# arindamrc/video_analytics

Hardware: AMD Instinct MI355X
Metric: clips/sec (224x224, RGB+10-flow two-stream) (higher is better)
Workload: dtype f32; 1 GPU; two-stream 224x224, 10-frame TV-L1 flow stack (5 scales x 5 warps x 300 its, fixed), VGG-16 spatial+temporal, batch=32 per GPU; global_batch=32, block_iters=0, tvl1_math=exact, flow_streams=2, batches_in_flight=1, tvl1_params=, tvl1_hip_blob=2e95b55cc558928abf4903d3eda147c92736cfdd, parallelism=clips sharded x1, finite=True

## Files before the change

video_analytics_amd/csrc/vgg.hip:

```cpp
#include "vgg_internal.h"
#include <cstdint>
#include <cstdlib>
#include <cstring>
#include <type_traits>

namespace {

typedef float f32x16 __attribute__((ext_vector_type(16)));
typedef float f32x4 __attribute__((ext_vector_type(4)));
typedef unsigned u32x4 __attribute__((ext_vector_type(4)));

template <int N, typename F>
__device__ __forceinline__ void static_for(F&& f)
{
    if constexpr (N > 0) {
        static_for<N - 1>(f);
        f(std::integral_constant<int, N - 1>{});
    }
}

constexpr int kBK = 16;
constexpr int kLdsStride = 20;


// ... 938 lines not shown
            constexpr int i = decltype(I)::value;
            if ((wave * PPW + i) < NPIECE) {
                const int y = Y0 + (pyx[i] >> 8) - 1, x = X0 + (pyx[i] & 255) - 1;
                const bool ok = pyx[i] >= 0 && y >= 0 && y < H && x >= 0 && x < W;
                __builtin_amdgcn_raw_ptr_buffer_load_lds(rs_a, (lds_ptr_t)(sA + buf * A_BYTES + (wave * PPW + i) * 1024), 16,
                                                         ok ? base + rel[i] : 0x7fffffff, 0, 0, 0);
            }
        });
    };

    const int r31 = lane & 31, hh = lane >> 5;
    int idx0[2], px0[2], py0[2];
#pragma unroll
    for (int mt = 0; mt < 2; ++mt) {
        int xl, yl, bl;
        brick_coords(64 * wave + 32 * mt + r31, 4, 4, xl, yl, bl);
        px0[mt] = xl + 1;
        py0[mt] = yl + 1;
        idx0[mt] = py0[mt] * PW + px0[mt];
    }
    const char* const wfrag = sW + r31 * WSTRIDE + hh * 16;

    if (first < aw.n_bricks) stage_a(first, 0);
    asm volatile("s_waitcnt vmcnt(0) lgkmcnt(0)" ::: "memory");
    __syncthreads();

    int buf = 0;
    for (int brick = first; brick < aw.n_bricks; brick += stride) {
        if (brick + stride < aw.n_bricks) stage_a(brick + stride, buf ^ 1);
        f32x16 acc[2][2];
#pragma unroll
        for (int mt = 0; mt < 2; ++mt)
#pragma unroll
            for (int nt = 0; nt < 2; ++nt)
#pragma unroll
                for (int r = 0; r < 16; ++r) acc[mt][nt][r] = 0.0f;
        const char* const pA = sA + buf * A_BYTES;
        bf16x8 fa[3][2], fb[3][2];
        auto fetch = [&](int i, int slot) __attribute__((always_inline)) {
            const int tap = i >> 2, ks = i & 3;
            const int toff = (tap / 3 - 1) * PW + (tap % 3) - 1;
#pragma unroll
            for (int mt = 0; mt < 2; ++mt) {
                const int row = idx0[mt] + toff;
                const int sw = (((px0[mt] + (tap % 3) - 1) >> 1) + 4 * (py0[mt] + tap / 3 - 1)) & 7;
                fa[slot][mt] = *reinterpret_cast<const bf16x8*>(pA + row * 128 + (((2 * ks + hh) ^ sw) << 4));
            }
#pragma unroll
            for (int nt = 0; nt < 2; ++nt)
                fb[slot][nt] = *reinterpret_cast<const bf16x8*>(wfrag + nt * 32 * WSTRIDE + (tap * 64 + ks * 16) * 2);
        };
        fetch(0, 0);
        fetch(1, 1);
#pragma unroll
        for (int i = 0; i < 36; ++i) {
            if (i + 2 < 36) fetch(i + 2, (i + 2) % 3);
            __builtin_amdgcn_sched_barrier(0);
#pragma unroll
            for (int mt = 0; mt < 2; ++mt)
#pragma unroll
                for (int nt = 0; nt < 2; ++nt)
                    acc[mt][nt] = kWeightsFirst<POOL> ? __builtin_amdgcn_mfma_f32_32x32x16_bf16(fb[i % 3][nt], fa[i % 3][mt], acc[mt][nt], 0, 0, 0)
                                                      : __builtin_amdgcn_mfma_f32_32x32x16_bf16(fa[i % 3][mt], fb[i % 3][nt], acc[mt][nt], 0, 0, 0);
            __builtin_amdgcn_sched_barrier(0);
        }
        asm volatile("s_waitcnt lgkmcnt(0)" ::: "memory");
        __builtin_amdgcn_s_barrier();
        {
            const int tx = brick % a.tiles_x, r1 = brick / a.tiles_x, ty = r1 % a.tiles_y, b = r1 / a.tiles_y;
            epilogue_lines_bf16<2, POOL>(acc, (__bf16*)(sA + buf * A_BYTES) + wave * 64 * 64, a, 64 * wave, nb, tx << 4, ty << 4, b, lane);
        }
        asm volatile("s_waitcnt vmcnt(0) lgkmcnt(0)" ::: "memory");
        __builtin_amdgcn_s_barrier();
        buf ^= 1;
    }
}

template <bool POOL>
__global__ void __launch_bounds__(256) k_conv3x3_ws_bf16(ConvArgsWs a)
{
    conv3x3_ws_body<POOL>(a);
}

struct Img14Args {
    const void* in;
    const void* wp;
    const float* bias;
    void* out;
    int B, Cin, Cout;
};

template <typename T, bool POOL>
__device__ __forceinline__ void conv3x3_img14_body(const Img14Args& a)
{
    constexpr bool F32 = sizeof(T) == 4;
    constexpr int EPC = 16 / (int)sizeof(T);
    constexpr int BK = 8 * EPC;
    constexpr int BRICK = 256 * BK, WT = 3 * 64 * BK, NWR = 3;
    constexpr int WPIECES = 6, BPIECES = 8;
    __shared__ __attribute__((aligned(1024))) T smem[2 * BRICK + NWR * WT];
    T* const sBrick = smem;
    T* const sW = smem + 2 * BRICK;
    const int tid = threadIdx.x, lane = tid & 63;
    const int wave8 = __builtin_amdgcn_readfirstlane(tid >> 6);
    const int wave = wave8 & 3;
    const int tiles_n = a.Cout / 64;
    const int n_tile = blockIdx.x % tiles_n, b = blockIdx.x / tiles_n;
    const int n0 = n_tile * 64, Cin = a.Cin;
    const int r31 = lane & 31, hh = lane >> 5, lrow = lane >> 3, lslot = lane & 7;
    const int nchunks = Cin / BK, NT_STEPS = 3 * nchunks;
    auto brick_swz = [](int bp) { return ((bp >> 1) & 3) | (((bp >> 4) & 1) << 2); };

    if (wave8 >= 4) {
        const T* const in = (const T*)a.in;
        const T* const wp = (const T*)a.wp;
        const __amdgpu_buffer_rsrc_t rs_a = __builtin_amdgcn_make_buffer_rsrc(
            const_cast<T*>(in) + (size_t)b * 196 * Cin, 0, 196 * Cin * (int)sizeof(T), 0x00020000);
        const __amdgpu_buffer_rsrc_t rs_b = __builtin_amdgcn_make_buffer_rsrc(
            const_cast<T*>(wp) + (size_t)n0 * 9 * Cin, 0, 64 * 9 * Cin * (int)sizeof(T), 0x00020000);
        int aoff[BPIECES];
#pragma unroll
        for (int i = 0; i < BPIECES; ++i) {
            const int bp = ((wave * 8 + i) << 3) + lrow, by = bp >> 4, bx = bp & 15;
            const bool ok = by >= 1 && by <= 14 && bx >= 1 && bx <= 14;
            aoff[i] = ok ? (((by - 1) * 14 + (bx - 1)) * Cin + EPC * (lslot ^ brick_swz(bp))) * (int)sizeof(T) : 0x7fffffff;
        }
        int boff[2];
#pragma unroll
        for (int i = 0; i < 2; ++i) {
            const int row = (wave * 2 + i) * 8 + lrow;
            boff[i] = (row * 9 * Cin + EPC * (lslot ^ ((row >> 1) & 7))) * (int)sizeof(T);
        }
        auto stage_brick = [&](int chunk) {
            T* const dst = sBrick + (chunk & 1) * BRICK;
            static_for<BPIECES>([&](auto I) {
                constexpr int i = decltype(I)::value;
                __builtin_amdgcn_raw_ptr_buffer_load_lds(rs_a, (lds_ptr_t)(dst + (wave * 8 + i) * 8 * BK), 16, aoff[i], chunk * BK * (int)sizeof(T), 0, 0);
            });
        };
        auto stage_w = [&](int t) {
            const int chunk = t / 3, ky = t - 3 * chunk;
            T* const dst = sW + (t % NWR) * WT;
            static_for<WPIECES>([&](auto I) {
                constexpr int i = decltype(I)::value, kx = i >> 1, h = i & 1;
                __builtin_amdgcn_raw_ptr_buffer_load_lds(rs_b, (lds_ptr_t)(dst + kx * 64 * BK + (wave * 2 + h) * 8 * BK), 16, boff[h],
                                                         ((3 * ky + kx) * Cin + chunk * BK) * (int)sizeof(T), 0, 0);
            });
        };
        stage_brick(0);
        stage_w(0);
        if (NT_STEPS > 1) stage_w(1);
        bool brick_prev = false;
        for (int t = 0; t < NT_STEPS; ++t) {
            const int chunk = t / 3, ky = t - 3 * chunk;
            if (t + 1 >= NT_STEPS) asm volatile("s_waitcnt vmcnt(0)" ::: "memory");
            else if (brick_prev) asm volatile("s_waitcnt vmcnt(14)" ::: "memory");
            else asm volatile("s_waitcnt vmcnt(6)" ::: "memory");
            __builtin_amdgcn_s_barrier();
            brick_prev = ky == 0 && chunk + 1 < nchunks;
            if (brick_prev) stage_brick(chunk + 1);
            if (t + 2 < NT_STEPS) stage_w(t + 2);
        }
        return;
    }

    constexpr int MT = 2, NT = 2;
    typedef typename std::conditional<F32, f32x4, bf16x8>::type frag_t;
    const int nrb = wave < 3 ? 2 : 1;
    int bp0[MT];
#pragma unroll
    for (int i = 0; i < MT; ++i) {
        const int qy = wave + 4 * i, qx = r31 >> 2;
        const int y = 2 * qy + ((r31 >> 1) & 1), x = 2 * qx + (r31 & 1);
        bp0[i] = (qx < 7 && qy < 7) ? (y + 1) * 16 + (x + 1) : 0;
    }
    f32x16 acc[MT][NT];
#pragma unroll
    for (int i = 0; i < MT; ++i)
#pragma unroll
        for (int j = 0; j < NT; ++j)
#pragma unroll
            for (int r = 0; r < 16; ++r) acc[i][j][r] = 0.0f;
    const int fsw = (r31 >> 1) & 7;
    auto mma = [&](const frag_t& fpix, const frag_t& fwgt, f32x16& c) __attribute__((always_inline)) {
        if constexpr (F32) {
#pragma unroll
            for (int e = 0; e < 4; ++e)
                c = POOL ? __builtin_amdgcn_mfma_f32_32x32x2f32(fpix[e], fwgt[e], c, 0, 0, 0) : __builtin_amdgcn_mfma_f32_32x32x2f32(fwgt[e], fpix[e], c, 0, 0, 0);
        } else {
            c = POOL ? __builtin_amdgcn_mfma_f32_32x32x16_bf16(fpix, fwgt, c, 0, 0, 0) : __builtin_amdgcn_mfma_f32_32x32x16_bf16(fwgt, fpix, c, 0, 0, 0);
        }
    };

    for (int t = 0; t < NT_STEPS; ++t) {
        const int chunk = t / 3, ky = t - 3 * chunk;
        asm volatile("s_waitcnt lgkmcnt(0)" ::: "memory");
        __builtin_amdgcn_s_barrier();
        const T* const sA = sBrick + (chunk & 1) * BRICK;
        const T* const sB = sW + (t % NWR) * WT;
        int arow[3][MT], asw[3][MT];
#pragma unroll
        for (int kx = 0; kx < 3; ++kx)
#pragma unroll
            for (int i = 0; i < MT; ++i) {
                const int bp = bp0[i] ? bp0[i] + (ky - 1) * 16 + (kx - 1) : 0;
                arow[kx][i] = bp * BK;
                asw[kx][i] = brick_swz(bp);
            }
        frag_t fa[2][2][MT], fb[2][2][NT];
        auto fetch = [&](auto SS, auto BUF) {
            constexpr int ss = decltype(SS)::value, kx = ss >> 1, bf = decltype(BUF)::value;
#pragma unroll
            for (int h = 0; h < 2; ++h) {
                const int ks = 2 * (ss & 1) + h;
#pragma unroll
                for (int i = 0; i < MT; ++i) fa[bf][h][i] = *reinterpret_cast<const frag_t*>(&sA[arow[kx][i] + (((2 * ks + hh) ^ asw[kx][i]) * EPC)]);
#pragma unroll
                for (int j = 0; j < NT; ++j)
                    fb[bf][h][j] = *reinterpret_cast<const frag_t*>(&sB[kx * 64 * BK + (j * 32 + r31) * BK + (((2 * ks + hh) ^ fsw) * EPC)]);
            }
        };
        fetch(std::integral_constant<int, 0>{}, std::integral_constant<int, 0>{});
        static_for<6>([&](auto SS) {
            constexpr int ss = decltype(SS)::value, cur = ss & 1;
            if constexpr (ss + 1 < 6) fetch(std::integral_constant<int, ss + 1>{}, std::integral_constant<int, cur ^ 1>{});
            __builtin_amdgcn_sched_barrier(0);
#pragma unroll
            for (int h = 0; h < 2; ++h)
#pragma unroll
                for (int i = 0; i < MT; ++i)
#pragma unroll
                    for (int j = 0; j < NT; ++j) mma(fa[cur][h][i], fb[cur][h][j], acc[i][j]);
            __builtin_amdgcn_sched_barrier(0);
        });
    }

    if constexpr (POOL) {
        float* const out = (float*)a.out + (size_t)b * 49 * a.Cout;
#pragma unroll
        for (int i = 0; i < MT; ++i) {
            if (i >= nrb) continue;
#pragma unroll
            for (int j = 0; j < NT; ++j) {
                const int n = n0 + 32 * j + r31;
                const float bias = a.bias[n];
#pragma unroll
                for (int g4 = 0; g4 < 4; ++g4) {
                    const int qy = wave + 4 * i, qx = 2 * g4 + hh;
                    if (qx >= 7 || qy >= 7) continue;
                    const int quad = 7 * qy + qx;
                    const float m01 = fmaxf(acc[i][j][4 * g4 + 0], acc[i][j][4 * g4 + 1]), m23 = fmaxf(acc[i][j][4 * g4 + 2], acc[i][j][4 * g4 + 3]);
                    out[(size_t)quad * a.Cout + n] = fmaxf(fmaxf(m01, m23) + bias, 0.0f);
                }
            }
        }
    } else {
        constexpr int NCHK = 64 / EPC;
        T* const stage = sBrick + (nchunks & 1) * BRICK + wave * 32 * 64;
        T* const out = (T*)a.out + (size_t)b * 196 * a.Cout + n0;
#pragma unroll
        for (int i = 0; i < MT; ++i) {
            if (i >= nrb) continue;
            const int qy = wave + 4 * i;
#pragma unroll
            for (int j = 0; j < NT; ++j)
#pragma unroll
                for (int g4 = 0; g4 < 4; ++g4) {
                    const int n = 32 * j + 8 * g4 + 4 * hh;
                    const float4 bs = *(const float4*)(a.bias + n0 + n);
                    const float v0 = fmaxf(acc[i][j][4 * g4 + 0] + bs.x, 0.0f), v1 = fmaxf(acc[i][j][4 * g4 + 1] + bs.y, 0.0f);
                    const float v2 = fmaxf(acc[i][j][4 * g4 + 2] + bs.z, 0.0f), v3 = fmaxf(acc[i][j][4 * g4 + 3] + bs.w, 0.0f);
                    T* const dst = stage + r31 * 64 + (((n / EPC) ^ (r31 & (NCHK - 1))) * EPC) + (n % EPC);
                    if constexpr (F32) {
                        *(float4*)dst = make_float4(v0, v1, v2, v3);
                    } else {
                        typedef __bf16 bf16x4 __attribute__((ext_vector_type(4)));
                        bf16x4 v;
                        v.x = (__bf16)v0, v.y = (__bf16)v1, v.z = (__bf16)v2, v.w = (__bf16)v3;
                        *(bf16x4*)dst = v;
                    }
                }
            __builtin_amdgcn_wave_barrier();
#pragma unroll
            for (int it = 0; it < 32 * NCHK / 64; ++it) {
                const int ch = it * 64 + lane, r = ch / NCHK, c8 = ch % NCHK, qx = r >> 2;
                const uint4 v = *(const uint4*)(stage + r * 64 + ((c8 ^ (r & (NCHK - 1))) * EPC));
                const int y = 2 * qy + ((r >> 1) & 1), x = 2 * qx + (r & 1);
                if (qx < 7) *(uint4*)(out + (size_t)(y * 14 + x) * a.Cout + EPC * c8) = v;
            }
            __builtin_amdgcn_wave_barrier();
        }
    }
}

template <typename T, bool POOL>
__global__ void __launch_bounds__(512) k_conv3x3_img14(Img14Args a)
{
    conv3x3_img14_body<T, POOL>(a);
}

constexpr int kDmaBK = 32;

template <int NT, bool POOL, int NBUF>
__global__ void __launch_bounds__(256, NBUF == 1 ? 4 : 2) k_conv3x3_dma_f32(ConvArgs a)
{
    constexpr int BM = 128, BN = NT * 64, MT = 2;
    constexpr int A_INSTR = BM / 32, B_INSTR = BN / 32;
    constexpr int TILE = (BM + BN) * kDmaBK;
    __shared__ __attribute__((aligned(1024))) float smem[NBUF * TILE];

    const int tid = threadIdx.x, lane = tid & 63, wave = tid >> 6;
    const int wm = wave >> 1, wn = wave & 1;
    int bid = xcd_remap(blockIdx.x, gridDim.x);
    const int n_tile = bid % a.tiles_n;
    bid /= a.tiles_n;
    const int tile_x = bid % a.tiles_x;
    bid /= a.tiles_x;
    const int tile_y = bid % a.tiles_y;
    const int tile_b = bid / a.tiles_y;
    const int n0 = n_tile * BN;
    const int H = a.H, W = a.W, Cin = a.Cin;
    const int X0 = tile_x << a.lgTW, Y0 = tile_y << a.lgTH, B0 = tile_b * a.TB;

    const int lrow = lane >> 3, lslot = lane & 7;
    int ax[A_INSTR], ay[A_INSTR];
    long apix[A_INSTR];
    bool aok[A_INSTR];
#pragma unroll
    for (int i = 0; i < A_INSTR; ++i) {
        const int row = (wave * A_INSTR + i) * 8 + lrow;
        const int c = lslot ^ ((row >> 1) & 7);
        int xl, yl, bl;
        brick_coords(row, a.lgTW, a.lgTH, xl, yl, bl);
        ax[i] = X0 + xl;
        ay[i] = Y0 + yl;
        const int b = B0 + bl;
        aok[i] = b < a.B && ax[i] < W && ay[i] < H;
        apix[i] = (((long)b * H + ay[i]) * W + ax[i]) * Cin + 4 * c;
    }
    const float* wrow[B_INSTR];
#pragma unroll
    for (int i = 0; i < B_INSTR; ++i) {
        const int row = (wave * B_INSTR + i) * 8 + lrow;
        wrow[i] = a.wp + (size_t)(n0 + row) * 9 * Cin + 4 * (lslot ^ ((row >> 1) & 7));
    }

    f32x16 acc[MT][NT];
#pragma unroll
    for (int mt = 0; mt < MT; ++mt)
#pragma unroll
        for (int nt = 0; nt < NT; ++nt)
#pragma unroll
            for (int r = 0; r < 16; ++r) acc[mt][nt][r] = 0.0f;

    const int cchunks = Cin / kDmaBK;
    const int T = 9 * cchunks;
    const int r31 = lane & 31, hh = lane >> 5;
    const int fsw = (r31 >> 1) & 7;
    int kp = 0, c0 = 0;
    auto stage = [&](int buf) {
        float* const sA = smem + buf * TILE;
        float* const sB = sA + BM * kDmaBK;
        const int ky = kp / 3 - 1, kx = kp % 3 - 1;
        const long tap = ((long)ky * W + kx) * Cin + c0;
        static_for<A_INSTR>([&](auto I) {
            constexpr int i = decltype(I)::value;
            const int yy = ay[i] + ky, xx = ax[i] + kx;
            const bool ok = aok[i] && yy >= 0 && yy < H && xx >= 0 && xx < W;
            const float* src = ok ? a.in + apix[i] + tap : a.zeros;
            __builtin_amdgcn_global_load_lds((gbl_ptr_t)src, (lds_ptr_t)(sA + (wave * A_INSTR + i) * 8 * kDmaBK), 16, 0, 0);
        });
        static_for<B_INSTR>([&](auto I) {
            constexpr int i = decltype(I)::value;
            __builtin_amdgcn_global_load_lds((gbl_ptr_t)(wrow[i] + (size_t)kp * Cin + c0),
                                             (lds_ptr_t)(sB + (wave * B_INSTR + i) * 8 * kDmaBK), 16, 0, 0);
        });
        c0 += kDmaBK;
        if (c0 == Cin) {
            c0 = 0;
            ++kp;
        }
    };
    auto compute = [&](int buf) {
        const float* const sA = smem + buf * TILE;
        const float* const sB = sA + BM * kDmaBK;
#pragma unroll
        for (int ks = 0; ks < kDmaBK / 8; ++ks) {
            f32x4 fa[MT], fb[NT];
            const int slot = ((2 * ks + hh) ^ fsw) * 4;
#pragma unroll
            for (int mt = 0; mt < MT; ++mt)
                fa[mt] = *reinterpret_cast<const f32x4*>(&sA[((wm * MT + mt) * 32 + r31) * kDmaBK + slot]);
#pragma unroll
            for (int nt = 0; nt < NT; ++nt)
                fb[nt] = *reinterpret_cast<const f32x4*>(&sB[((wn * NT + nt) * 32 + r31) * kDmaBK + slot]);
#pragma unroll
            for (int j = 0; j < 4; ++j)
#pragma unroll
                for (int mt = 0; mt < MT; ++mt)
#pragma unroll
                    for (int nt = 0; nt < NT; ++nt)
                        acc[mt][nt] = __builtin_amdgcn_mfma_f32_32x32x2f32(fa[mt][j], fb[nt][j], acc[mt][nt], 0, 0, 0);
        }
    };
    if constexpr (NBUF == 1) {
        for (int t = 0; t < T; ++t) {
            stage(0);
            asm volatile("s_waitcnt vmcnt(0)" ::: "memory");
            __syncthreads();
            compute(0);
            __syncthreads();
        }
    } else {
        constexpr int LOADS = A_INSTR + B_INSTR;
        for (int j = 0; j < NBUF - 1 && j < T; ++j) stage(j);
        int slot = 0;
        for (int t = 0; t < T; ++t) {
            if (t + NBUF - 2 < T) {
                if constexpr ((NBUF - 2) * LOADS == 6) asm volatile("s_waitcnt vmcnt(6)" ::: "memory");
                else if constexpr ((NBUF - 2) * LOADS == 8) asm volatile("s_waitcnt vmcnt(8)" ::: "memory");
                else if constexpr ((NBUF - 2) * LOADS == 12) asm volatile("s_waitcnt vmcnt(12)" ::: "memory");
                else if constexpr ((NBUF - 2) * LOADS == 16) asm volatile("s_waitcnt vmcnt(16)" ::: "memory");
                else asm volatile("s_waitcnt vmcnt(0)" ::: "memory");
            } else {
                asm volatile("s_waitcnt vmcnt(0)" ::: "memory");
            }
            asm volatile("s_waitcnt lgkmcnt(0)" ::: "memory");
            __builtin_amdgcn_s_barrier();
            if (t + NBUF - 1 < T) stage(slot == 0 ? NBUF - 1 : slot - 1);
            compute(slot);
            slot = slot + 1 == NBUF ? 0 : slot + 1;
        }
    }

#pragma unroll
    for (int nt = 0; nt < NT; ++nt) {
        const int n = n0 + (wn * NT + nt) * 32 + r31;
        const float bias = a.bias[n];
#pragma unroll
        for (int mt = 0; mt < MT; ++mt) {
#pragma unroll
            for (int g4 = 0; g4 < 4; ++g4) {
                const int mbase = (wm * MT + mt) * 32 + 8 * g4 + 4 * hh;
                int xl, yl, bl;
                brick_coords(mbase, a.lgTW, a.lgTH, xl, yl, bl);
                const int x = X0 + xl, y = Y0 + yl, b = B0 + bl;
                if (b >= a.B) continue;
                float v[4];
#pragma unroll
                for (int j = 0; j < 4; ++j) {
                    v[j] = acc[mt][nt][4 * g4 + j] + bias;
                    if (!a.linear) v[j] = fmaxf(v[j], 0.0f);
                }
                if constexpr (POOL) {
                    if (x < W && y < H) {
                        const float mx = fmaxf(fmaxf(v[0], v[1]), fmaxf(v[2], v[3]));
                        a.out[((((size_t)b * (H >> 1)) + (y >> 1)) * (W >> 1) + (x >> 1)) * a.Cout + n] = mx;
                    }
                } else {
#pragma unroll
                    for (int j = 0; j < 4; ++j) {
                        const int xx = x + (j & 1), yy = y + (j >> 1);
                        if (xx < W && yy < H) {
                            const size_t o = (((size_t)b * H + yy) * W + xx) * a.Cout + n;
                            a.out[o] = (a.mask && !(a.mask[o] > 0.0f)) ? 0.0f : v[j];
                        }
                    }
                }
            }
        }
    }
}



struct FcArgs {
    const float* A;
    const float* Wt;
    float* slab;
    int M, N, K, S, kchunk, Npad;
};

constexpr int kFcDepth = 4;
__global__ void __launch_bounds__(256) k_fc_splitk(FcArgs a)
{
    __shared__ __attribute__((aligned(16))) float sA[2][32 * kLdsStride];
    __shared__ __attribute__((aligned(16))) float sB[2][128 * kLdsStride];
    const int tid = threadIdx.x, lane = tid & 63, wave = tid >> 6;
    const int ntiles = a.Npad / 128;
    const int n_tile = blockIdx.x % ntiles, s = blockIdx.x / ntiles;
    const int m0 = blockIdx.y * 32, n0 = n_tile * 128;
    const int k0 = s * a.kchunk;
    const int kend = (k0 + a.kchunk < a.K) ? k0 + a.kchunk : a.K;
    const int T = (kend - k0) / kBK;
    const int q = tid & 3, rowbase = tid >> 2;

    const bool a_loader = rowbase < 32;
    const int am = m0 + (rowbase & 31);
    const float* arow = a.A + (size_t)(am < a.M ? am : 0) * a.K + 4 * q;
    const float* brow[2];
#pragma unroll
    for (int i = 0; i < 2; ++i) {
        const int n = n0 + rowbase + 64 * i;
        brow[i] = a.Wt + (size_t)(n < a.N ? n : 0) * a.K + 4 * q;
    }
    f32x16 acc;
#pragma unroll
    for (int r = 0; r < 16; ++r) acc[r] = 0.0f;
    f32x4 ra[kFcDepth], rb[kFcDepth][2];
    const int tlast = T > 0 ? T - 1 : 0;
    auto gload = [&](auto jc, int t) {
        constexpr int j = decltype(jc)::value;
        const int k = k0 + (t < tlast ? t : tlast) * kBK;
        ra[j] = *reinterpret_cast<const f32x4*>(arow + k);
#pragma unroll
        for (int i = 0; i < 2; ++i) rb[j][i] = *reinterpret_cast<const f32x4*>(brow[i] + k);
    };
    auto lstore = [&](auto jc, int buf) {
        constexpr int j = decltype(jc)::value;
        if (a_loader) *reinterpret_cast<f32x4*>(&sA[buf][rowbase * kLdsStride + 4 * q]) = ra[j];
#pragma unroll
        for (int i = 0; i < 2; ++i) *reinterpret_cast<f32x4*>(&sB[buf][(rowbase + 64 * i) * kLdsStride + 4 * q]) = rb[j][i];
    };
    const int r31 = lane & 31, hh = lane >> 5;
    if (T <= 0) return;
    static_for<kFcDepth>([&](auto jc) { gload(jc, jc.value); });
    lstore(std::integral_constant<int, 0>{}, 0);
    gload(std::integral_constant<int, 0>{}, kFcDepth);
    __syncthreads();
    auto body = [&](auto jc, int t) {
        constexpr int jn = (decltype(jc)::value + 1) % kFcDepth;
        const int buf = t & 1;
#pragma unroll
        for (int g = 0; g < 2; ++g) {
            const float4 fa = *reinterpret_cast<const float4*>(&sA[buf][r31 * kLdsStride + 8 * g + 4 * hh]);
            const float4 fb = *reinterpret_cast<const float4*>(&sB[buf][(wave * 32 + r31) * kLdsStride + 8 * g + 4 * hh]);
            acc = __builtin_amdgcn_mfma_f32_32x32x2f32(fa.x, fb.x, acc, 0, 0, 0);
            acc = __builtin_amdgcn_mfma_f32_32x32x2f32(fa.y, fb.y, acc, 0, 0, 0);
            acc = __builtin_amdgcn_mfma_f32_32x32x2f32(fa.z, fb.z, acc, 0, 0, 0);
            acc = __builtin_amdgcn_mfma_f32_32x32x2f32(fa.w, fb.w, acc, 0, 0, 0);
        }
        lstore(std::integral_constant<int, jn>{}, buf ^ 1);
        gload(std::integral_constant<int, jn>{}, t + 1 + kFcDepth);
        __syncthreads();
    };
    int t = 0;
    for (; t + kFcDepth <= T; t += kFcDepth)
        static_for<kFcDepth>([&](auto jc) { body(jc, t + jc.value); });
    static_for<kFcDepth>([&](auto jc) {
        if (t + jc.value < T) body(jc, t + jc.value);
    });
    const int n = n0 + wave * 32 + r31;
    const size_t Mp = (size_t)gridDim.y * 32;
#pragma unroll
    for (int r = 0; r < 16; ++r) {
        const int m = m0 + (r & 3) + 8 * (r >> 2) + 4 * hh;
        a.slab[((size_t)s * Mp + m) * a.Npad + n] = acc[r];
    }
}

__global__ void k_fc_reduce(const float* __restrict__ slab, const float* __restrict__ bias, float* __restrict__ out,
                            int M, int N, int Npad, int Mp, int S, int relu)
{
    const int idx = blockIdx.x * blockDim.x + threadIdx.x;
    if (idx >= M * N) return;
    const int m = idx / N, n = idx - m * N;
    float acc = bias[n];
    for (int s = 0; s < S; ++s) acc += slab[((size_t)s * Mp + m) * Npad + n];
    out[idx] = relu ? fmaxf(acc, 0.0f) : acc;
}

__global__ void k_validate_batch(const float* __restrict__ logits, const long long* __restrict__ labels, int B, int C,
                                 float* __restrict__ out)
{
    __shared__ float sloss[256];
    __shared__ int scorr[256];
    float loss = 0.0f;
    int corr = 0;
    for (int b = threadIdx.x; b < B; b += blockDim.x) {
        const float* l = logits + (size_t)b * C;
        float mx = l[0];
        int am = 0;
        for (int c = 1; c < C; ++c)
            if (l[c] > mx) { mx = l[c]; am = c; }
        float se = 0.0f;
        for (int c = 0; c < C; ++c) se += expf(l[c] - mx);
        const long long y = labels[b];
        const bool yok = y >= 0 && y < (long long)C;
        loss += yok ? (logf(se) + mx) - l[yok ? y : 0] : __builtin_nanf("");
        corr += (yok && am == (int)y);
    }
    sloss[threadIdx.x] = loss;
    scorr[threadIdx.x] = corr;
    __syncthreads();
    if (threadIdx.x == 0) {
        float L = 0.0f;
        int Cc = 0;
        for (int i = 0; i < (int)blockDim.x; ++i) { L += sloss[i]; Cc += scorr[i]; }
        out[0] = L / (float)B;
        out[1] = (float)Cc;
    }
}


constexpr int kConvCout[13] = {64, 64, 128, 128, 256, 256, 256, 512, 512, 512, 512, 512, 512};
constexpr bool kConvPool[13] = {false, true, false, true, false, false, true, false, false, true, false, false, true};

}

namespace {

constexpr long VA_WIDE_MIN = 512;
constexpr int VA_RING = 3;
constexpr long VA_RING_MAXGRID = 1024;
constexpr long VA_RING_MAXGRID_F32 = 1024;
constexpr const char* kRetiredVariant6 =
    "6 selected a retired VA_EXPERIMENTS kernel family (k_conv3x3_bpp_bf16): measured no faster and removed, see DESIGN.md section 7; commit "
    "eebd154 is the last one that contains it";
constexpr int VA_F32_CONV_DEFAULT = 1;
constexpr int VA_CIN_ALIGN = 16;

void pick_brick(int W, int H, int B, int& lgTW, int& lgTH, int& TB, int lgpx = 7)
{
    double best = -1.0;
    for (int lw = 1; lw <= 5; ++lw)
        for (int lh = 1; lw + lh <= lgpx; ++lh) {
            const int tw = 1 << lw, th = 1 << lh, tb = (1 << lgpx) / (tw * th);
            const double cover = (double)va_cdiv(W, tw) * tw * va_cdiv(H, th) * th * (double)va_cdiv(B, tb) * tb;
            double util = (double)W * H * B / cover;
            util += 1e-3 * lw;
            if (lgpx != 7) util += 5e-4 * lh;
            if (util > best) {
                best = util;
                lgTW = lw;
                lgTH = lh;
                TB = tb;
            }
        }
}

#define VA_LAUNCHED(name_)                 \
    do {                                   \
        if (launched) *launched = (name_); \
    } while (0)
static_assert(VA_RING == 3, "the launched-kernel names below spell the ring depth");

int launch_conv_ex(int hw, int cin_pad, int cout, const float* wp, const float* bias, const float* in, float* out,
                   const float* mask, int linear, bool pool, int B, const float* zeros, int f32_conv, hipStream_t st,
                   const char** launched = nullptr)
{
    ConvArgs a{};
    a.in = in;
    a.wp = wp;
    a.bias = bias;
    a.out = out;
    a.mask = mask;
    a.linear = linear;
    a.zeros = zeros;
    a.B = B;
    a.H = a.W = hw;
    a.Cin = cin_pad;
    a.Cout = cout;
    pick_brick(hw, hw, B, a.lgTW, a.lgTH, a.TB);
    a.tiles_x = va_cdiv(hw, 1 << a.lgTW);
    a.tiles_y = va_cdiv(hw, 1 << a.lgTH);
    const int tiles_b = va_cdiv(B, a.TB);
    if (f32_conv == 1 && hw == 14 && mask == nullptr && !linear && cin_pad % 32 == 0 && cout % 64 == 0) {
        const Img14Args ia{in, wp, bias, out, B, cin_pad, cout};
        const unsigned gridi = (unsigned)(B * (cout / 64));
        if (pool) k_conv3x3_img14<float, true><<<gridi, 512, 0, st>>>(ia);
        else k_conv3x3_img14<float, false><<<gridi, 512, 0, st>>>(ia);
        VA_LAUNCHED(pool ? "k_conv3x3_img14<float,true>" : "k_conv3x3_img14<float,false>");
        VA_LAUNCH_CHECK();
        return VA_OK;
    }
    if (f32_conv == 1 && zeros != nullptr && cin_pad % kDmaBK == 0) {
        const long grid64 = (long)(cout / 64) * a.tiles_x * a.tiles_y * tiles_b;
        const int ksteps = 9 * (cin_pad / kDmaBK);
        const bool ring = grid64 < VA_RING_MAXGRID_F32 && ksteps >= VA_RING;
        const bool wide = !ring && cout % 128 == 0;
        a.tiles_n = cout / (wide ? 128 : 64);
        const unsigned grid = (unsigned)(a.tiles_n * a.tiles_x * a.tiles_y * tiles_b);
#define VA_LAUNCH_F32(NT_, NB_)                                                                                      \
    {                                                                                                                \
        if (pool) k_conv3x3_dma_f32<NT_, true, NB_><<<grid, 256, 0, st>>>(a);                                        \
        else k_conv3x3_dma_f32<NT_, false, NB_><<<grid, 256, 0, st>>>(a);                                            \
        VA_LAUNCHED(pool ? "k_conv3x3_dma_f32<" #NT_ ",true," #NB_ ">" : "k_conv3x3_dma_f32<" #NT_ ",false," #NB_ ">"); \
    }
        if (ring) VA_LAUNCH_F32(1, 3)
        else if (wide) VA_LAUNCH_F32(2, 1)
        else VA_LAUNCH_F32(1, 1)
#undef VA_LAUNCH_F32
        VA_LAUNCH_CHECK();
        return VA_OK;
    }
    const bool wide = cout % 128 == 0 && (long)(cout / 128) * a.tiles_x * a.tiles_y * tiles_b >= VA_WIDE_MIN;
    if (wide) {
        a.tiles_n = cout / 128;
        const unsigned grid = (unsigned)(a.tiles_n * a.tiles_x * a.tiles_y * tiles_b);
        if (pool) k_conv3x3_mfma<2, 2, 2, 2, true, 16><<<grid, 256, 0, st>>>(a);
        else k_conv3x3_mfma<2, 2, 2, 2, false, 16><<<grid, 256, 0, st>>>(a);
        VA_LAUNCHED(pool ? "k_conv3x3_mfma<2,2,2,2,true,16>" : "k_conv3x3_mfma<2,2,2,2,false,16>");
    } else {
        a.tiles_n = cout / 64;
        const unsigned grid = (unsigned)(a.tiles_n * a.tiles_x * a.tiles_y * tiles_b);
        if (pool) k_conv3x3_mfma<2, 2, 2, 1, true, 16><<<grid, 256, 0, st>>>(a);
        else k_conv3x3_mfma<2, 2, 2, 1, false, 16><<<grid, 256, 0, st>>>(a);
        VA_LAUNCHED(pool ? "k_conv3x3_mfma<2,2,2,1,true,16>" : "k_conv3x3_mfma<2,2,2,1,false,16>");
    }
    VA_LAUNCH_CHECK();
    return VA_OK;
}

int launch_conv(const ConvLayer& L, const float* zeros, const float* in, float* out, int B, int f32_conv, hipStream_t st)
{
    return launch_conv_ex(L.hw, L.cin_pad, L.cout, L.wp, L.bias, in, out, nullptr, 0, L.pool, B, zeros, f32_conv, st);
}

int launch_conv_bf16(const ConvLayer& L, const __bf16* zeros, int variant, const __bf16* in, void* out, bool out_f32, int B, int n_cu,
                     hipStream_t st, const char** launched = nullptr)
{
    ConvArgsBf a{};
    a.in = in;
    a.zeros = zeros;
    a.taps_x = L.xcol ? 1 : 3;
    a.wp = L.wp_bf;
    a.bias = L.bias;
    a.out = out;
    a.B = B;
    a.H = a.W = L.hw;
    a.Cin = L.cin_pad;
    a.Cout = L.cout;
    VA_CHECK_ARG(((long)B * L.hw * L.hw + 2L * (L.hw + 1)) * L.cin_pad * 2 < 2147483647L,
                 "va_vgg16_forward (bf16): batch %d x %dx%dx%d activations exceed 2 GiB of 32-bit buffer offsets: split the batch", B,
                 L.hw, L.hw, L.cin_pad);
    pick_brick(L.hw, L.hw, B, a.lgTW, a.lgTH, a.TB);
    a.tiles_x = va_cdiv(L.hw, 1 << a.lgTW);
    a.tiles_y = va_cdiv(L.hw, 1 << a.lgTH);
    const int tiles_b = va_cdiv(B, a.TB);
    bool pp = !L.xcol && !out_f32 && a.Cin % 32 == 0 && L.cout % 128 == 0 && L.hw >= 28 && (variant == 5 || variant == 0);
    if (pp) {
        int lw, lh, tb;
        pick_brick(L.hw, L.hw, B, lw, lh, tb, 8);
        const bool nt4 = L.cout % 256 == 0;
        const long gridp = (long)(L.cout / (nt4 ? 256 : 128)) * va_cdiv(L.hw, 1 << lw) * va_cdiv(L.hw, 1 << lh) * va_cdiv(B, tb);
        if (variant == 0) pp = nt4 && ((gridp >= 160 && gridp <= 256) || gridp >= 1024);
    }
    if (pp) {
        pick_brick(L.hw, L.hw, B, a.lgTW, a.lgTH, a.TB, 8);
        a.tiles_x = va_cdiv(L.hw, 1 << a.lgTW);
        a.tiles_y = va_cdiv(L.hw, 1 << a.lgTH);
        const bool nt4 = L.cout % 256 == 0;
        a.tiles_n = L.cout / (nt4 ? 256 : 128);
        const unsigned gridp = (unsigned)(a.tiles_n * a.tiles_x * a.tiles_y * va_cdiv(B, a.TB));
        if (nt4) {
            if (L.pool) k_conv3x3_pp_bf16<4, true><<<gridp, 512, 0, st>>>(a);
            else k_conv3x3_pp_bf16<4, false><<<gridp, 512, 0, st>>>(a);
            VA_LAUNCHED(L.pool ? "k_conv3x3_pp_bf16<4,true>" : "k_conv3x3_pp_bf16<4,false>");
        } else {
            if (L.pool) k_conv3x3_pp_bf16<2, true><<<gridp, 512, 0, st>>>(a);
            else k_conv3x3_pp_bf16<2, false><<<gridp, 512, 0, st>>>(a);
            VA_LAUNCHED(L.pool ? "k_conv3x3_pp_bf16<2,true>" : "k_conv3x3_pp_bf16<2,false>");
        }
        VA_LAUNCH_CHECK();
        return VA_OK;
    }
    if ((variant == 0 || variant >= 5) && !L.xcol && L.hw == 14 && a.Cin % 64 == 0 && L.cout % 64 == 0 &&
        (long)B * (L.cout / 64) <= 65535L * 16 && ((out_f32 && L.pool) || (!out_f32 && !L.pool))) {
        const unsigned gridi = (unsigned)(B * (L.cout / 64));
        const Img14Args ia{a.in, a.wp, a.bias, a.out, B, a.Cin, a.Cout};
        if (out_f32) k_conv3x3_img14<__bf16, true><<<gridi, 512, 0, st>>>(ia);
        else k_conv3x3_img14<__bf16, false><<<gridi, 512, 0, st>>>(ia);
        VA_LAUNCHED(out_f32 ? "k_conv3x3_img14<__bf16,true>" : "k_conv3x3_img14<__bf16,false>");
        VA_LAUNCH_CHECK();
        return VA_OK;
    }
    if ((variant == 7 || (variant == 0 && L.cout == 64)) && !L.xcol && !out_f32 && a.Cin == 64 && L.cout % 64 == 0 &&
        L.cout <= 256 && L.hw % 16 == 0 && n_cu >= L.cout / 64) {
        ConvArgsWs w{};
        w.c = a;
        w.c.lgTW = w.c.lgTH = 4;
        w.c.TB = 1;
        w.c.tiles_x = w.c.tiles_y = L.hw / 16;
        w.n_bricks = B * w.c.tiles_x * w.c.tiles_y;
        const int nh = L.cout / 64;
        const unsigned gridw = (unsigned)((n_cu / nh) * nh);
        if (L.pool) k_conv3x3_ws_bf16<true><<<gridw, 256, 0, st>>>(w);
        else k_conv3x3_ws_bf16<false><<<gridw, 256, 0, st>>>(w);
        VA_LAUNCHED(L.pool ? "k_conv3x3_ws_bf16<true>" : "k_conv3x3_ws_bf16<false>");
        VA_LAUNCH_CHECK();
        return VA_OK;
    }
    const long grid64 = (long)(L.cout / 64) * a.tiles_x * a.tiles_y * tiles_b;
    const int ksteps = 3 * a.taps_x * (a.Cin / 64);
    const bool autosel = variant == 0 || variant >= 5;
    const bool ring = autosel ? (grid64 < VA_RING_MAXGRID && ksteps >= VA_RING) : (variant == 2 && ksteps >= VA_RING);
    const bool wide = autosel && !ring && L.cout % 128 == 0;
    a.tiles_n = L.cout / (wide ? 128 : 64);
    const unsigned grid = (unsigned)(a.tiles_n * a.tiles_x * a.tiles_y * tiles_b);
#define VA_LAUNCH_BF(NT_, NB_)                                                                                  \
    {                                                                                                           \
        if (out_f32) k_conv3x3_mfma_bf16<NT_, true, true, NB_><<<grid, 256, 0, st>>>(a);                        \
        else if (L.pool) k_conv3x3_mfma_bf16<NT_, true, false, NB_><<<grid, 256, 0, st>>>(a);                   \
        else k_conv3x3_mfma_bf16<NT_, false, false, NB_><<<grid, 256, 0, st>>>(a);                              \
        VA_LAUNCHED(out_f32  ? "k_conv3x3_mfma_bf16<" #NT_ ",true,true," #NB_ ">"                                \
                    : L.pool ? "k_conv3x3_mfma_bf16<" #NT_ ",true,false," #NB_ ">"                               \
                             : "k_conv3x3_mfma_bf16<" #NT_ ",false,false," #NB_ ">");                            \
    }
    if (ring) VA_LAUNCH_BF(1, 3)
    else if (wide) VA_LAUNCH_BF(2, 1)
    else VA_LAUNCH_BF(1, 1)
#undef VA_LAUNCH_BF
    VA_LAUNCH_CHECK();
    return VA_OK;
}
#undef VA_LAUNCHED

struct FcPlan {
    int S, kchunk, Npad, Mtiles;
    size_t slab_floats;
};

FcPlan plan_fc(int M, int N, int K)
{
    FcPlan p;
    p.Npad = va_cdiv(N, 128) * 128;
    p.Mtiles = va_cdiv(M, 32);
    const int ntiles = p.Npad / 128;
    int S = va_cdiv(512, ntiles * p.Mtiles);
    int maxS = K / 256;
    if (maxS < 1) maxS = 1;
    if (S > maxS) S = maxS;
    if (S < 1) S = 1;
    p.kchunk = va_cdiv(va_cdiv(K, S), kBK) * kBK;
    p.S = va_cdiv(K, p.kchunk);
    p.slab_floats = (size_t)p.S * p.Mtiles * 32 * p.Npad;
    return p;
}

int launch_fc(const float* A, const float* Wt, const float* bias, float* out, float* slab, int M, int N, int K,
              bool relu, hipStream_t st)
{
    const FcPlan p = plan_fc(M, N, K);
    FcArgs a{};
    a.A = A;
    a.Wt = Wt;
    a.slab = slab;
    a.M = M;
    a.N = N;
    a.K = K;
    a.S = p.S;
    a.kchunk = p.kchunk;
    a.Npad = p.Npad;
    const dim3 grid((unsigned)((p.Npad / 128) * p.S), (unsigned)p.Mtiles);
    k_fc_splitk<<<grid, 256, 0, st>>>(a);
    k_fc_reduce<<<va_cdiv(M * N, 256), 256, 0, st>>>(slab, bias, out, M, N, p.Npad, p.Mtiles * 32, p.S, relu ? 1 : 0);
    VA_LAUNCH_CHECK();
    return VA_OK;
}

struct WsPlan {
    size_t off_act[2], off_slab, off_fc[2], total;
};

WsPlan plan_ws(const va_vgg16* m, int B)
{
    WsPlan w;
    size_t off = 0;
    const size_t act = va_align_up((size_t)B * 224 * 224 * 64 * sizeof(float), 256);
    w.off_act[0] = off; off += act;
    w.off_act[1] = off; off += act;
    size_t slab = 0;
    for (int i = 0; i < 4; ++i) {
        const FcPlan p = plan_fc(B, m->fc_out[i], m->fc_in[i]);
        if (p.slab_floats > slab) slab = p.slab_floats;
    }
    w.off_slab = off; off += va_align_up(slab * sizeof(float), 256);
    const size_t fc = va_align_up((size_t)B * 4096 * sizeof(float), 256);
    w.off_fc[0] = off; off += fc;
    w.off_fc[1] = off; off += fc;
    w.total = off;
    return w;
}

}

int va_conv3x3_f32(int hw, int cin_pad, int cout, const float* wp, const float* bias, const float* in, float* out,
                   const float* mask, int linear, int pool, int B, const float* zeros, int f32_conv, hipStream_t st, const char** launched)
{
    return launch_conv_ex(hw, cin_pad, cout, wp, bias, in, out, mask, linear, pool != 0, B, zeros, f32_conv, st, launched);
}

int va_fc_f32(const float* A, const float* Wt, const float* bias, float* out, float* slab, int M, int N, int K, int relu, hipStream_t st)
{
    return launch_fc(A, Wt, bias, out, slab, M, N, K, relu != 0, st);
}

size_t va_fc_slab_floats(int M, int N, int K) { return plan_fc(M, N, K).slab_floats; }

extern "C" int va_conv3x3_layer(va_ctx* ctx, int dtype, int kernel_opt, int hw, int cin_pad, int cout, int pool, int linear,
                                int out_f32, int batch, const void* in, const void* w_packed, const float* bias, const float* mask,
                                const void* zeros, void* out, char* kernel_name, int name_len, void* stream)
{
    VA_CHECK_ARG(ctx != nullptr, "va_conv3x3_layer: ctx is NULL");
    VA_USE_DEVICE(ctx);
    if (kernel_name && name_len > 0) kernel_name[0] = 0;
    VA_CHECK_ARG(in && w_packed && bias && zeros && out, "va_conv3x3_layer: NULL in/w_packed/bias/zeros/out");
    VA_CHECK_ARG((((uintptr_t)in | (uintptr_t)w_packed | (uintptr_t)bias | (uintptr_t)zeros | (uintptr_t)out | (uintptr_t)mask) & 15) == 0,
                 "va_conv3x3_layer: every pointer must be 16-byte aligned (16-byte vector accesses)");
    VA_CHECK_ARG(dtype == VA_DTYPE_F32 || dtype == VA_DTYPE_BF16, "va_conv3x3_layer: dtype must be VA_DTYPE_F32 or VA_DTYPE_BF16");
    const bool bf = dtype == VA_DTYPE_BF16;
    VA_CHECK_ARG(!(bf && kernel_opt == 6), "va_conv3x3_layer: bf16 kernel_opt %s", kRetiredVariant6);
    if (bf)
        VA_CHECK_ARG((kernel_opt >= 0 && kernel_opt <= 2) || kernel_opt == 5 || kernel_opt == 7,
                     "va_conv3x3_layer: bf16 kernel_opt (VA_OPT_BF16_VARIANT) must be 0, 1, 2, 5 or 7");
    else
        VA_CHECK_ARG(kernel_opt == 0 || kernel_opt == 1, "va_conv3x3_layer: fp32 kernel_opt (VA_OPT_F32_CONV_KERNEL) must be 0 or 1");
    VA_CHECK_ARG(batch >= 1, "va_conv3x3_layer: batch %d < 1", batch);
    VA_CHECK_ARG(hw >= 1, "va_conv3x3_layer: hw %d < 1", hw);
    VA_CHECK_ARG(bf ? cin_pad >= 64 && cin_pad % 64 == 0 : cin_pad >= 16 && cin_pad % 16 == 0,
                 "va_conv3x3_layer: cin_pad %d must be a positive multiple of %d", cin_pad, bf ? 64 : 16);
    VA_CHECK_ARG(cout >= 64 && cout % 64 == 0, "va_conv3x3_layer: cout %d must be a positive multiple of 64", cout);
    VA_CHECK_ARG(pool == 0 || pool == 1, "va_conv3x3_layer: pool must be 0 or 1");
    VA_CHECK_ARG(!pool || hw % 2 == 0, "va_conv3x3_layer: pooling needs an even hw (got %d)", hw);
    VA_CHECK_ARG(!out_f32 || (bf && pool), "va_conv3x3_layer: out_f32 needs dtype bf16 and pool");
    VA_CHECK_ARG(!linear || !bf, "va_conv3x3_layer: linear (no ReLU) is an fp32-only form (training dgrad)");
    VA_CHECK_ARG(mask == nullptr || (!bf && !pool), "va_conv3x3_layer: mask needs dtype fp32 and no pool");
    VA_CHECK_ARG((long)batch * hw * hw * cin_pad < 2147483647L && (long)batch * hw * hw * cout < 2147483647L,
                 "va_conv3x3_layer: %d x %d x %d x %d/%d activations exceed 2^31 elements", batch, hw, hw, cin_pad, cout);
    VA_CHECK_ARG((long)cout * 9 * cin_pad * (bf ? 2 : 4) < 2147483647L, "va_conv3x3_layer: packed weights exceed 2 GiB");
    hipStream_t st = (hipStream_t)stream;
    const char* name = nullptr;
    int rc;
    if (bf) {
        ConvLayer L{};
        L.cin = L.cin_pad = cin_pad;
        L.cout = cout;
        L.hw = hw;
        L.pool = pool != 0;
        L.xcol = false;
        L.wp_bf = (__bf16*)w_packed;
        L.bias = (float*)bias;
        rc = launch_conv_bf16(L, (const __bf16*)zeros, kernel_opt, (const __bf16*)in, out, out_f32 != 0, batch, ctx->n_cu, st, &name);
    } else {
        rc = launch_conv_ex(hw, cin_pad, cout, (const float*)w_packed, bias, (const float*)in, (float*)out, mask, linear, pool != 0,
                            batch, (const float*)zeros, kernel_opt, st, &name);
    }
    if (rc == VA_OK && kernel_name && name_len > 0) snprintf(kernel_name, (size_t)name_len, "%s", name ? name : "");
    return rc;
}

int va_input_to_nhwc_f32(const va_vgg16* m, const void* x, int x_is_u8, int B, float* out, hipStream_t st)
{
    const int HW0 = 224 * 224;
    const unsigned pgrid = (unsigned)(B * ((HW0 + 63) / 64));
    if (x_is_u8)
        k_nchw_to_nhwc_pad<unsigned char, float><<<pgrid, 256, 0, st>>>((const unsigned char*)x, out, B, m->c_in, HW0, m->c_in_pad, m->in_mean, m->in_std);
    else
        k_nchw_to_nhwc_pad<float, float><<<pgrid, 256, 0, st>>>((const float*)x, out, B, m->c_in, HW0, m->c_in_pad, nullptr, nullptr);
    VA_LAUNCH_CHECK();
    return VA_OK;
}

static int run_classifier(va_vgg16* m, const float* f, int B, void* desc, void* logits, float* slab, float* const* fcbuf,
                          hipStream_t st)
{
    if (int rc = launch_fc(f, m->fcw[0], m->fcb[0], fcbuf[0], slab, B, 4096, 512 * 49, true, st)) return rc;
    if (int rc = launch_fc(fcbuf[0], m->fcw[1], m->fcb[1], fcbuf[1], slab, B, 4096, 4096, true, st)) return rc;
    float* d = desc ? (float*)desc : fcbuf[0];
    if (int rc = launch_fc(fcbuf[1], m->fcw[2], m->fcb[2], d, slab, B, m->desc_dim, 4096, true, st)) return rc;
    if (logits)
        if (int rc = launch_fc(d, m->fcw[3], m->fcb[3], (float*)logits, slab, B, m->n_classes, m->desc_dim, false, st)) return rc;
    return VA_OK;
}

extern "C" int va_vgg16_create(va_ctx* ctx, int c_in, int n_classes, int desc_dim, int dtype,
                               const void* const* conv_w, const void* const* conv_b, const void* const* fc_w,
                               const void* const* fc_b, const float* in_mean, const float* in_std, void* stream,
                               va_vgg16** out)
// ... 322 lines not shown
```

Measured before the change: 262.3 clips/s.

## Use buffer-resource LDS loads with precomputed tap masks and software-pipelined LDS fragment fetch in f32 conv

Replaces per-tap 64-bit pointer arithmetic and zero-pointer selects in the f32 DMA conv kernel with buffer resource descriptors, 32-bit offsets and a precomputed 9-bit validity mask. Out-of-range rows get an all-ones offset so the buffer range check drops the load. It also double-buffers the LDS fragment reads across k-substeps with sched barriers, and overlaps next-step address prep with the final MFMA group. A host guard rejects shapes whose offsets could overflow 32 bits. The goal is lower VALU/SALU address overhead and better MFMA/LDS overlap, at the cost of more registers and reliance on buffer OOB semantics.

```diff
diff --git a/video_analytics_amd/csrc/vgg.hip b/video_analytics_amd/csrc/vgg.hip
--- a/video_analytics_amd/csrc/vgg.hip
+++ b/video_analytics_amd/csrc/vgg.hip
@@ -1264,14 +1264,15 @@
 constexpr int kDmaBK = 32;
 
 template <int NT, bool POOL, int NBUF>
-__global__ void __launch_bounds__(256, NBUF == 1 ? 4 : 2) k_conv3x3_dma_f32(ConvArgs a)
+__device__ __forceinline__ void conv3x3_dma_f32_body(const ConvArgs& a)
 {
     constexpr int BM = 128, BN = NT * 64, MT = 2;
     constexpr int A_INSTR = BM / 32, B_INSTR = BN / 32;
     constexpr int TILE = (BM + BN) * kDmaBK;
     __shared__ __attribute__((aligned(1024))) float smem[NBUF * TILE];
 
-    const int tid = threadIdx.x, lane = tid & 63, wave = tid >> 6;
+    const int tid = threadIdx.x, lane = tid & 63;
+    const int wave = __builtin_amdgcn_readfirstlane(tid >> 6);
     const int wm = wave >> 1, wn = wave & 1;
     int bid = xcd_remap(blockIdx.x, gridDim.x);
     const int n_tile = bid % a.tiles_n;
@@ -1285,26 +1286,33 @@
     const int X0 = tile_x << a.lgTW, Y0 = tile_y << a.lgTH, B0 = tile_b * a.TB;
 
     const int lrow = lane >> 3, lslot = lane & 7;
-    int ax[A_INSTR], ay[A_INSTR];
-    long apix[A_INSTR];
-    bool aok[A_INSTR];
+    const __amdgpu_buffer_rsrc_t rs_a = __builtin_amdgcn_make_buffer_rsrc(
+        const_cast<float*>(a.in) + ((((long)B0 * H + Y0) * W + X0) - (W + 1)) * Cin, 0, 0x7fffffff, 0x00020000);
+    const __amdgpu_buffer_rsrc_t rs_b = __builtin_amdgcn_make_buffer_rsrc(
+        const_cast<float*>(a.wp) + (size_t)n0 * 9 * Cin, 0, BN * 9 * Cin * 4, 0x00020000);
+    int arel[A_INSTR], amask[A_INSTR];
 #pragma unroll
     for (int i = 0; i < A_INSTR; ++i) {
         const int row = (wave * A_INSTR + i) * 8 + lrow;
         const int c = lslot ^ ((row >> 1) & 7);
         int xl, yl, bl;
         brick_coords(row, a.lgTW, a.lgTH, xl, yl, bl);
-        ax[i] = X0 + xl;
-        ay[i] = Y0 + yl;
-        const int b = B0 + bl;
-        aok[i] = b < a.B && ax[i] < W && ay[i] < H;
-        apix[i] = (((long)b * H + ay[i]) * W + ax[i]) * Cin + 4 * c;
-    }
-    const float* wrow[B_INSTR];
+        const int x = X0 + xl, y = Y0 + yl;
+        const bool ok = B0 + bl < a.B && x < W && y < H;
+        arel[i] = ok ? (((bl * H + yl) * W + xl) * Cin + 4 * c) * 4 : 0;
+        int m = 0;
+#pragma unroll
+        for (int k = 0; k < 9; ++k) {
+            const int yy = y + k / 3 - 1, xx = x + k % 3 - 1;
+            if (ok && yy >= 0 && yy < H && xx >= 0 && xx < W) m |= 1 << k;
+        }
+        amask[i] = m;
+    }
+    int woff[B_INSTR];
 #pragma unroll
     for (int i = 0; i < B_INSTR; ++i) {
         const int row = (wave * B_INSTR + i) * 8 + lrow;
-        wrow[i] = a.wp + (size_t)(n0 + row) * 9 * Cin + 4 * (lslot ^ ((row >> 1) & 7));
+        woff[i] = (row * 9 * Cin + 4 * (lslot ^ ((row >> 1) & 7))) * 4;
     }
 
     f32x16 acc[MT][NT];
@@ -1320,62 +1328,75 @@
     const int r31 = lane & 31, hh = lane >> 5;
     const int fsw = (r31 >> 1) & 7;
     int kp = 0, c0 = 0;
-    auto stage = [&](int buf) {
-        float* const sA = smem + buf * TILE;
-        float* const sB = sA + BM * kDmaBK;
-        const int ky = kp / 3 - 1, kx = kp % 3 - 1;
-        const long tap = ((long)ky * W + kx) * Cin + c0;
-        static_for<A_INSTR>([&](auto I) {
-            constexpr int i = decltype(I)::value;
-            const int yy = ay[i] + ky, xx = ax[i] + kx;
-            const bool ok = aok[i] && yy >= 0 && yy < H && xx >= 0 && xx < W;
-            const float* src = ok ? a.in + apix[i] + tap : a.zeros;
-            __builtin_amdgcn_global_load_lds((gbl_ptr_t)src, (lds_ptr_t)(sA + (wave * A_INSTR + i) * 8 * kDmaBK), 16, 0, 0);
-        });
-        static_for<B_INSTR>([&](auto I) {
-            constexpr int i = decltype(I)::value;
-            __builtin_amdgcn_global_load_lds((gbl_ptr_t)(wrow[i] + (size_t)kp * Cin + c0),
-                                             (lds_ptr_t)(sB + (wave * B_INSTR + i) * 8 * kDmaBK), 16, 0, 0);
-        });
+    int avo[A_INSTR], so_a, so_b;
+    auto prep = [&]() __attribute__((always_inline)) {
+#pragma unroll
+        for (int i = 0; i < A_INSTR; ++i) avo[i] = arel[i] | (int)(((unsigned)amask[i] >> kp & 1u) - 1u);
+        so_a = (((kp / 3) * W + kp % 3) * Cin + c0) * 4;
+        so_b = (kp * Cin + c0) * 4;
         c0 += kDmaBK;
         if (c0 == Cin) {
             c0 = 0;
             ++kp;
         }
     };
-    auto compute = [&](int buf) {
-        const float* const sA = smem + buf * TILE;
-        const float* const sB = sA + BM * kDmaBK;
-#pragma unroll
-        for (int ks = 0; ks < kDmaBK / 8; ++ks) {
-            f32x4 fa[MT], fb[NT];
-            const int slot = ((2 * ks + hh) ^ fsw) * 4;
-#pragma unroll
-            for (int mt = 0; mt < MT; ++mt)
-                fa[mt] = *reinterpret_cast<const f32x4*>(&sA[((wm * MT + mt) * 32 + r31) * kDmaBK + slot]);
-#pragma unroll
-            for (int nt = 0; nt < NT; ++nt)
-                fb[nt] = *reinterpret_cast<const f32x4*>(&sB[((wn * NT + nt) * 32 + r31) * kDmaBK + slot]);
+    auto issue = [&](int buf) __attribute__((always_inline)) {
+        float* const sA = smem + buf * TILE;
+        float* const sB = sA + BM * kDmaBK;
+        static_for<A_INSTR>([&](auto I) {
+            constexpr int i = decltype(I)::value;
+            __builtin_amdgcn_raw_ptr_buffer_load_lds(rs_a, (lds_ptr_t)(sA + (wave * A_INSTR + i) * 8 * kDmaBK), 16, avo[i], so_a, 0, 0);
+        });
+        static_for<B_INSTR>([&](auto I) {
+            constexpr int i = decltype(I)::value;
+            __builtin_amdgcn_raw_ptr_buffer_load_lds(rs_b, (lds_ptr_t)(sB + (wave * B_INSTR + i) * 8 * kDmaBK), 16, woff[i], so_b, 0, 0);
+        });
+    };
+    constexpr int KS = kDmaBK / 8;
+    int fa0 = (((wm * MT) * 32 + r31) * kDmaBK + (hh ^ fsw) * 4) * 4, fb0 = (((wn * NT) * 32 + r31) * kDmaBK + (hh ^ fsw) * 4) * 4;
+    f32x4 fa[2][MT], fb[2][NT];
+    auto fetch = [&](int buf, auto KSI) __attribute__((always_inline)) {
+        constexpr int ks = decltype(KSI)::value, set = ks & 1;
+        const char* const sA = (const char*)(smem + buf * TILE);
+        const char* const sB = sA + BM * kDmaBK * 4;
+#pragma unroll
+        for (int mt = 0; mt < MT; ++mt) fa[set][mt] = *reinterpret_cast<const f32x4*>(sA + (fa0 ^ (32 * ks)) + mt * 32 * kDmaBK * 4);
+#pragma unroll
+        for (int nt = 0; nt < NT; ++nt) fb[set][nt] = *reinterpret_cast<const f32x4*>(sB + (fb0 ^ (32 * ks)) + nt * 32 * kDmaBK * 4);
+    };
+    auto compute = [&](int buf, auto&& early) __attribute__((always_inline)) {
+        static_for<KS>([&](auto KSI) {
+            constexpr int ks = decltype(KSI)::value, set = ks & 1;
+            if constexpr (ks + 1 < KS) fetch(buf, std::integral_constant<int, ks + 1>{});
+            if constexpr (ks + 1 == KS) early();
+            __builtin_amdgcn_sched_barrier(0);
 #pragma unroll
             for (int j = 0; j < 4; ++j)
 #pragma unroll
                 for (int mt = 0; mt < MT; ++mt)
 #pragma unroll
                     for (int nt = 0; nt < NT; ++nt)
-                        acc[mt][nt] = __builtin_amdgcn_mfma_f32_32x32x2f32(fa[mt][j], fb[nt][j], acc[mt][nt], 0, 0, 0);
-        }
+                        acc[mt][nt] = __builtin_amdgcn_mfma_f32_32x32x2f32(fa[set][mt][j], fb[set][nt][j], acc[mt][nt], 0, 0, 0);
+            __builtin_amdgcn_sched_barrier(0);
+        });
     };
     if constexpr (NBUF == 1) {
+        static_assert(A_INSTR == 4, "the second barrier's operand list");
+        prep();
         for (int t = 0; t < T; ++t) {
-            stage(0);
-            asm volatile("s_waitcnt vmcnt(0)" ::: "memory");
-            __syncthreads();
-            compute(0);
-            __syncthreads();
+            issue(0);
+            asm volatile("s_waitcnt vmcnt(0)\n\ts_barrier" ::: "memory");
+            asm volatile("" : "+v"(fa0), "+v"(fb0));
+            fetch(0, std::integral_constant<int, 0>{});
+            compute(0, [&]() __attribute__((always_inline)) { prep(); });
+            asm volatile("s_waitcnt lgkmcnt(0)\n\ts_barrier" : "+v"(avo[0]), "+v"(avo[1]), "+v"(avo[2]), "+v"(avo[3])::"memory");
         }
     } else {
         constexpr int LOADS = A_INSTR + B_INSTR;
-        for (int j = 0; j < NBUF - 1 && j < T; ++j) stage(j);
+        for (int j = 0; j < NBUF - 1 && j < T; ++j) {
+            prep();
+            issue(j);
+        }
         int slot = 0;
         for (int t = 0; t < T; ++t) {
             if (t + NBUF - 2 < T) {
@@ -1387,10 +1408,13 @@
             } else {
                 asm volatile("s_waitcnt vmcnt(0)" ::: "memory");
             }
-            asm volatile("s_waitcnt lgkmcnt(0)" ::: "memory");
-            __builtin_amdgcn_s_barrier();
-            if (t + NBUF - 1 < T) stage(slot == 0 ? NBUF - 1 : slot - 1);
-            compute(slot);
+            asm volatile("s_waitcnt lgkmcnt(0)\n\ts_barrier" ::: "memory");
+            fetch(slot, std::integral_constant<int, 0>{});
+            if (t + NBUF - 1 < T) {
+                prep();
+                issue(slot == 0 ? NBUF - 1 : slot - 1);
+            }
+            compute(slot, []() {});
             slot = slot + 1 == NBUF ? 0 : slot + 1;
         }
     }
@@ -1432,6 +1456,12 @@
             }
         }
     }
+}
+
+template <int NT, bool POOL, int NBUF>
+__global__ void __launch_bounds__(256, NBUF == 1 ? 4 : 2) k_conv3x3_dma_f32(ConvArgs a)
+{
+    conv3x3_dma_f32_body<NT, POOL, NBUF>(a);
 }
 
 
@@ -1637,6 +1667,7 @@
         return VA_OK;
     }
     if (f32_conv == 1 && zeros != nullptr && cin_pad % kDmaBK == 0) {
+        if (((long)a.TB * hw + (1L << a.lgTH) + 4) * (hw + 32) * cin_pad * 4 >= 2147483647L) return VA_ERR_INVALID;
         const long grid64 = (long)(cout / 64) * a.tiles_x * a.tiles_y * tiles_b;
         const int ksteps = 9 * (cin_pad / kDmaBK);
         const bool ring = grid64 < VA_RING_MAXGRID_F32 && ksteps >= VA_RING;
```

Result: faster. 265.3 clips/s, median of 6 (+1.2%).
